# WestlyPark/StyleRenderer

Measured on AMD Instinct MI355X. Metric: generator fwd+bwd images/sec at 256^2, higher is better.
Workload: dtype f32

## Files before the change

stylerenderer_amd/csrc/conv1x1_gemm.h:

```cpp
#pragma once
#include <hip/hip_runtime.h>
#include <stdint.h>

bool sr_conv1x1_gemm_eligible(int64_t B, int64_t C, int64_t N, int64_t ldw, int64_t P, const void* in, const void* wt,
                              const void* out);
int sr_conv1x1_gemm_launch(float* out, const float* in, const float* wt, int64_t ldw, const float* iscale,
                           const float* oscale, const float* obias, int64_t B, int64_t C, int64_t N, int64_t P,
                           hipStream_t st, const float* addend = nullptr);

bool sr_convt_taps_gemm_eligible(int64_t B, int64_t C, int64_t N, int64_t IW, int64_t ldw, int c_per_slice,
                                 const void* wt);
int sr_convt_taps_gemm_launch(float* partial, const float* in, const float* wt, int64_t ldw, const float* iscale, int64_t B,
                              int64_t C, int64_t N, int64_t IH, int64_t IW, int ks, int c_per_slice, hipStream_t st);
```

stylerenderer_amd/csrc/conv1x1_gemm.hip:

```cpp
#include "mfma_tile.h"
#include "conv1x1_gemm.h"

#include <cstdlib>

namespace {

constexpr int TN = 128, TP = 128, KC = 16;

struct GemmParams {
    const float* x;
    const float* wt;
    const float* iscale;
    const float* oscale;
    const float* obias;
    const float* addend;
    float* out;
    int C, N, ldw;
    int64_t P;
    int tiles_p, tiles_n;
};

__global__ __launch_bounds__(256, 2) void k_conv1x1_gemm(const GemmParams q) {
#if __HIP_DEVICE_COMPILE__
    __shared__ float s_a[2][KC][TN];
    __shared__ float s_b[2][KC][TP];
    int bid = blockIdx.x;
    const int tp = bid % q.tiles_p;
    bid /= q.tiles_p;
    const int tn = bid % q.tiles_n;
    const int b = bid / q.tiles_n;
    const int n0 = tn * TN;
    const int64_t p0 = (int64_t)tp * TP;
    const int tid = threadIdx.x, lane = tid & 63, wave = tid >> 6;
    const int l31 = lane & 31, half = lane >> 5;
    const int wn = (wave >> 1) * 64, wp = (wave & 1) * 64;

    const int r0 = tid >> 5, c4 = (tid & 31) * 4;
    const float* wsrc = q.wt + (int64_t)r0 * q.ldw + n0 + c4;
    const float* xsrc = q.x + ((int64_t)b * q.C + r0) * q.P + p0 + c4;
    const float* isc = q.iscale ? q.iscale + (int64_t)b * q.C : nullptr;
    const int64_t wstep8 = (int64_t)8 * q.ldw, xstep8 = (int64_t)8 * q.P;

    f32x16 acc[2][2];
#pragma unroll
    for (int i = 0; i < 2; ++i)
#pragma unroll
        for (int j = 0; j < 2; ++j)
#pragma unroll
            for (int r = 0; r < 16; ++r) acc[i][j][r] = 0.0f;

    float4 ra0, ra1, rb0, rb1;
    auto fetch = [&](int kc) {
        const float* w = wsrc + (int64_t)kc * KC * q.ldw;
        const float* xx = xsrc + (int64_t)kc * KC * q.P;
        ra0 = *reinterpret_cast<const float4*>(w);
        ra1 = *reinterpret_cast<const float4*>(w + wstep8);
        rb0 = *reinterpret_cast<const float4*>(xx);
        rb1 = *reinterpret_cast<const float4*>(xx + xstep8);
        if (isc) {
            const float s0 = isc[kc * KC + r0], s1 = isc[kc * KC + r0 + 8];
            rb0.x *= s0; rb0.y *= s0; rb0.z *= s0; rb0.w *= s0;
            rb1.x *= s1; rb1.y *= s1; rb1.z *= s1; rb1.w *= s1;
        }
    };
    auto stash = [&](int buf) {
        *reinterpret_cast<float4*>(&s_a[buf][r0][c4]) = ra0;
        *reinterpret_cast<float4*>(&s_a[buf][r0 + 8][c4]) = ra1;
        *reinterpret_cast<float4*>(&s_b[buf][r0][c4]) = rb0;
        *reinterpret_cast<float4*>(&s_b[buf][r0 + 8][c4]) = rb1;
    };

    const int nchunks = q.C / KC;
    fetch(0);
    stash(0);
    __syncthreads();
    for (int kc = 0; kc < nchunks; ++kc) {
        const int buf = kc & 1;
        const bool more = kc + 1 < nchunks;
        if (more) fetch(kc + 1);
#pragma unroll
        for (int kk = 0; kk < KC / 2; ++kk) {
            const int k = 2 * kk + half;
            const float a0 = s_a[buf][k][wn + l31], a1 = s_a[buf][k][wn + 32 + l31];
            const float b0 = s_b[buf][k][wp + l31], b1 = s_b[buf][k][wp + 32 + l31];
            acc[0][0] = __builtin_amdgcn_mfma_f32_32x32x2f32(a0, b0, acc[0][0], 0, 0, 0);
            acc[0][1] = __builtin_amdgcn_mfma_f32_32x32x2f32(a0, b1, acc[0][1], 0, 0, 0);
            acc[1][0] = __builtin_amdgcn_mfma_f32_32x32x2f32(a1, b0, acc[1][0], 0, 0, 0);
            acc[1][1] = __builtin_amdgcn_mfma_f32_32x32x2f32(a1, b1, acc[1][1], 0, 0, 0);
        }
        if (more) stash(buf ^ 1);
        __syncthreads();
    }

    float* dst = q.out + ((int64_t)b * q.N + n0 + wn) * q.P + p0 + wp + l31;
    const float* osc = q.oscale ? q.oscale + (int64_t)b * q.N + n0 + wn : nullptr;
    const float* bia = q.obias ? q.obias + n0 + wn : nullptr;
#pragma unroll
    for (int i = 0; i < 2; ++i)
#pragma unroll
        for (int r = 0; r < 16; ++r) {
            const int row = sr_mfma32_row(r, half, i * 32);
            const float s = osc ? osc[row] : 1.0f;
            const float t = bia ? bia[row] : 0.0f;
            float* d = dst + (int64_t)row * q.P;
            float v0 = acc[i][0][r] * s + t, v1 = acc[i][1][r] * s + t;
            if (q.addend) {
                const float* a = q.addend + (d - q.out);
                v0 += a[0];
                v1 += a[32];
            }
            d[0] = v0;
            d[32] = v1;
        }
#endif
}

struct TapParams {
    const float* x;
    const float* wt;
    const float* iscale;
    float* partial;
    int B, C, N, ldw, IH, IW, GW, region;
    int tiles_q, tiles_n, c_per_slice;
    int64_t total_q;
};

__global__ __launch_bounds__(256, 2) void k_convt_taps_gemm(const TapParams q) {
#if __HIP_DEVICE_COMPILE__
    __shared__ float s_a[2][KC][TN];
    __shared__ float s_b[2][KC][TP];
    int bid = blockIdx.x;
    const int tap = bid % 9;
    bid /= 9;
    const int tn = bid % q.tiles_n;
    bid /= q.tiles_n;
    const int tq = bid % q.tiles_q;
    const int slice = bid / q.tiles_q;
    const int c_beg = slice * q.c_per_slice;
    const int c_end = min(q.C, c_beg + q.c_per_slice);
    const int n0 = tn * TN;
    const int tid = threadIdx.x, lane = tid & 63, wave = tid >> 6;
    const int l31 = lane & 31, half = lane >> 5;
    const int wn = (wave >> 1) * 64, wp = (wave & 1) * 64;
    const int ky = tap / 3, kx = tap - 3 * ky;

    const int r0 = tid >> 5, c4 = (tid & 31) * 4;
    const float* wsrc = q.wt + ((int64_t)tap * q.C + c_beg + r0) * q.ldw + n0 + c4;
    const int64_t wstep8 = (int64_t)8 * q.ldw;
    const int col = tid & 127, rb0 = tid >> 7;
    const int64_t qi = (int64_t)tq * TP + col;
    const int plane = q.IH * q.IW;
    bool ok = qi < q.total_q;
    const int bq = ok ? (int)(qi / q.region) : 0;
    const int g = ok ? (int)(qi - (int64_t)bq * q.region) : 0;
    const int yy = g / q.GW - (ky >> 1), xx = g % q.GW - (kx >> 1);
    ok = ok && yy >= 0 && yy < q.IH && xx >= 0 && xx < q.IW;
    const float* xsrc = q.x + ((int64_t)bq * q.C + c_beg + rb0) * plane + (ok ? yy * q.IW + xx : 0);
    const float* isc = q.iscale ? q.iscale + (int64_t)bq * q.C + c_beg + rb0 : nullptr;

    f32x16 acc[2][2];
#pragma unroll
    for (int i = 0; i < 2; ++i)
#pragma unroll
        for (int j = 0; j < 2; ++j)
#pragma unroll
            for (int r = 0; r < 16; ++r) acc[i][j][r] = 0.0f;

    float4 ra0, ra1;
    float rb[8];
    auto fetch = [&](int kc) {
        const float* w = wsrc + (int64_t)kc * KC * q.ldw;
        ra0 = *reinterpret_cast<const float4*>(w);
        ra1 = *reinterpret_cast<const float4*>(w + wstep8);
        const float* xx_ = xsrc + (int64_t)kc * KC * plane;
#pragma unroll
        for (int i = 0; i < 8; ++i) {
            float v = ok ? xx_[(int64_t)(2 * i) * plane] : 0.0f;
            if (isc) v *= isc[kc * KC + 2 * i];
            rb[i] = v;
        }
    };
    auto stash = [&](int buf) {
        *reinterpret_cast<float4*>(&s_a[buf][r0][c4]) = ra0;
        *reinterpret_cast<float4*>(&s_a[buf][r0 + 8][c4]) = ra1;
#pragma unroll
        for (int i = 0; i < 8; ++i) s_b[buf][rb0 + 2 * i][col] = rb[i];
    };

    const int nchunks = (c_end - c_beg) / KC;
    if (nchunks > 0) {
        fetch(0);
        stash(0);
    }
    __syncthreads();
    for (int kc = 0; kc < nchunks; ++kc) {
        const int buf = kc & 1;
        const bool more = kc + 1 < nchunks;
        if (more) fetch(kc + 1);
#pragma unroll
        for (int kk = 0; kk < KC / 2; ++kk) {
            const int k = 2 * kk + half;
            const float a0 = s_a[buf][k][wn + l31], a1 = s_a[buf][k][wn + 32 + l31];
            const float b0 = s_b[buf][k][wp + l31], b1 = s_b[buf][k][wp + 32 + l31];
            acc[0][0] = __builtin_amdgcn_mfma_f32_32x32x2f32(a0, b0, acc[0][0], 0, 0, 0);
            acc[0][1] = __builtin_amdgcn_mfma_f32_32x32x2f32(a0, b1, acc[0][1], 0, 0, 0);
            acc[1][0] = __builtin_amdgcn_mfma_f32_32x32x2f32(a1, b0, acc[1][0], 0, 0, 0);
            acc[1][1] = __builtin_amdgcn_mfma_f32_32x32x2f32(a1, b1, acc[1][1], 0, 0, 0);
        }
        if (more) stash(buf ^ 1);
        __syncthreads();
    }

    float* base = q.partial + ((int64_t)slice * 9 + tap) * q.B * q.N * q.region;
#pragma unroll
    for (int j = 0; j < 2; ++j) {
        const int64_t qo = (int64_t)tq * TP + wp + j * 32 + l31;
        if (qo >= q.total_q) continue;
        const int bo = (int)(qo / q.region);
        const int go = (int)(qo - (int64_t)bo * q.region);
        float* d = base + ((int64_t)bo * q.N + n0 + wn) * q.region + go;
#pragma unroll
        for (int i = 0; i < 2; ++i)
#pragma unroll
            for (int r = 0; r < 16; ++r) {
                const int row = sr_mfma32_row(r, half, i * 32);
                d[(int64_t)row * q.region] = acc[i][j][r];
            }
    }
#endif
}

int mode() {
    const int e = sr_env_char("SR_CONV1X1_GEMM");
    return e == '0' ? 0 : (e == 'f' ? 2 : 1);
}

}

bool sr_conv1x1_gemm_eligible(int64_t B, int64_t C, int64_t N, int64_t ldw, int64_t P, const void* in, const void* wt,
                              const void* out) {
    const int m = mode();
    if (m == 0 || B <= 0) return false;
    if (C % KC != 0 || N % TN != 0 || P % TP != 0 || ldw % 4 != 0) return false;
    if (((reinterpret_cast<uintptr_t>(in) | reinterpret_cast<uintptr_t>(wt) | reinterpret_cast<uintptr_t>(out)) & 15) != 0)
        return false;
    const int64_t tiles = (P / TP) * (N / TN) * B;
    return (m == 2 || tiles >= SR_NUM_CU) && tiles < (1LL << 31);
}

int sr_conv1x1_gemm_launch(float* out, const float* in, const float* wt, int64_t ldw, const float* iscale,
                           const float* oscale, const float* obias, int64_t B, int64_t C, int64_t N, int64_t P,
                           hipStream_t st, const float* addend) {
    GemmParams q;
    q.x = in; q.wt = wt; q.iscale = iscale; q.oscale = oscale; q.obias = obias; q.out = out; q.addend = addend;
    q.C = (int)C; q.N = (int)N; q.ldw = (int)ldw; q.P = P;
    q.tiles_p = (int)(P / TP); q.tiles_n = (int)(N / TN);
    const int64_t tiles = (int64_t)q.tiles_p * q.tiles_n * B;
    hipLaunchKernelGGL(k_conv1x1_gemm, dim3((unsigned)tiles), dim3(256), 0, st, q);
    return sr_launch_status();
}

bool sr_convt_taps_gemm_eligible(int64_t B, int64_t C, int64_t N, int64_t IW, int64_t ldw, int c_per_slice,
                                 const void* wt) {
    const int e = sr_env_char("SR_CONVT_TAPS_GEMM");
    if (e == '0') return false;
    if (IW > 32 && e != 'f') return false;
    return B > 0 && C % KC == 0 && c_per_slice % KC == 0 && N % TN == 0 && ldw % 4 == 0 &&
           (reinterpret_cast<uintptr_t>(wt) & 15) == 0;
}

int sr_convt_taps_gemm_launch(float* partial, const float* in, const float* wt, int64_t ldw, const float* iscale, int64_t B,
                              int64_t C, int64_t N, int64_t IH, int64_t IW, int ks, int c_per_slice, hipStream_t st) {
    TapParams q;
    q.x = in; q.wt = wt; q.iscale = iscale; q.partial = partial;
    q.B = (int)B; q.C = (int)C; q.N = (int)N; q.ldw = (int)ldw; q.IH = (int)IH; q.IW = (int)IW;
    q.GW = (int)IW + 1; q.region = (int)((IH + 1) * (IW + 1));
    q.total_q = B * q.region;
    q.tiles_q = (int)((q.total_q + TP - 1) / TP); q.tiles_n = (int)(N / TN); q.c_per_slice = c_per_slice;
    const int64_t blocks = (int64_t)q.tiles_q * q.tiles_n * 9 * ks;
    if (blocks > 0x7FFFFFFFLL) return SR_ERANGE;
    hipLaunchKernelGGL(k_convt_taps_gemm, dim3((unsigned)blocks), dim3(256), 0, st, q);
    return sr_launch_status();
}

extern "C" int sr_conv1x1_add_supported(int64_t B, int64_t C, int64_t N, int64_t wt_ld, int64_t P, const float* in,
                                        const float* wt, const float* out, const float* addend) {
    return sr_conv1x1_gemm_eligible(B, C, N, wt_ld, P, in, wt, out) && (reinterpret_cast<uintptr_t>(addend) & 15) == 0 ? 1 : 0;
}

extern "C" int sr_conv1x1_add(float* out, const float* in, const float* wt, const float* oscale, const float* addend,
                              int64_t B, int64_t C, int64_t N, int64_t wt_ld, int64_t P, sr_stream_t stream) {
    if (!out || !in || !wt || !addend) return SR_EINVAL;
    if (!sr_conv1x1_add_supported(B, C, N, wt_ld, P, in, wt, out, addend)) return SR_EINVAL;
    if (B * C * P >= (1LL << 31)) return SR_ERANGE;
    return sr_conv1x1_gemm_launch(out, in, wt, wt_ld, nullptr, oscale, nullptr, B, C, N, P, sr_stream(stream), addend);
}
```

stylerenderer_amd/csrc/conv_mfma.hip:

```cpp
#include "conv_mfma.h"

#include "conv1x1_gemm.h"
#include "mfma_tile.h"

#include <algorithm>
#include <cstdlib>

namespace {

constexpr int BN = 128;
constexpr int BM = 128;

__device__ __attribute__((aligned(16))) const float g_zero_line[4] = {0.f, 0.f, 0.f, 0.f};
__device__ __attribute__((aligned(16))) const float g_ones_line[4] = {1.f, 1.f, 1.f, 1.f};

template <int IS, int TY, int TX, int PW, int PH, int PB, bool V4, bool TAP9 = false>
struct Geo {
    static constexpr bool ROT = V4 && IS == 2;
    static constexpr int NT = TY * TX;
    static constexpr int KC = NT >= 9 ? 4 : (NT >= 4 ? 8 : 16);
    static constexpr int EH = (PH - 1) * IS + TY;
    static constexpr int EW = (PW - 1) * IS + TX;
    static constexpr int LEAD = (V4 && !ROT) ? (TAP9 ? 4 : (TX > 1 ? 3 : 0)) : 0;
    static constexpr int EWP = ROT ? (EW + 3 + 3) / 4 * 4
                                   : (V4 ? (LEAD + EW + 3) / 4 * 4 : EW + ((EW % 2 == 0) ? 1 : 0));
    static constexpr int PLANE = PB * EH * EWP;
    static constexpr int W_FLOATS = NT * KC * BN;
    static constexpr int W_INSTR = W_FLOATS / 256;
    static constexpr int IMG_INSTR = V4 ? (KC * PLANE + 255) / 256 : 0;
    static constexpr int ST_INSTR = V4 ? (KC * PB + 63) / 64 : 0;
    static constexpr int IN_FLOATS = KC * PLANE + KC * PB;
    static constexpr int IN_INSTR = V4 ? IMG_INSTR + ST_INSTR : (IN_FLOATS + 63) / 64;
    static constexpr int S_BASE = V4 ? W_FLOATS + IMG_INSTR * 256 : W_FLOATS + KC * PLANE;
    static constexpr int BUF = V4 ? S_BASE + ST_INSTR * 64 : W_FLOATS + IN_INSTR * 64;
    static constexpr int W_PER_WAVE = (W_INSTR + 3) / 4;
    static constexpr int IN_PER_WAVE = (IN_INSTR + 3) / 4;
    static constexpr int LDS_BYTES = 2 * BUF * 4;
};

template <int IS, int TY, int TX, int PW, int PH, int PB, bool V4, bool FAST, bool TAP9 = false>
__global__ __launch_bounds__(256) void k_conv_mfma(const ConvParams p) {
    using G = Geo<IS, TY, TX, PW, PH, PB, V4, TAP9>;
    static_assert(PW * PH * PB == BM, "patch must hold 128 pixels");
    static_assert(!TAP9 || (IS == 1 && TY == 1 && TX == 1), "tap-split mode is a shifted 1x1 convolution");
    extern __shared__ __attribute__((aligned(16))) float smem[];

    int bid = sr_xcd_chunk(blockIdx.x, gridDim.x);
    int tap = 0, g_dy0 = p.dy0, g_dx0 = p.dx0, g_gh = p.GH, g_gw = p.GW, g_ooy = p.ooy, g_oox = p.oox, g_slab = p.wmap[0];
    int tap_local = 0;
    if (TAP9) {
        tap_local = bid % p.tap_count;
        bid /= p.tap_count;
        tap = p.tap_first + tap_local * p.tap_step;
        const int ky = tap / 3, kx = tap - 3 * ky;
        g_dy0 = -(ky >> 1); g_dx0 = -(kx >> 1);
        g_ooy = ky & 1; g_oox = kx & 1;
        g_gh = min(g_ooy ? p.IH : p.IH + 1, p.GH); g_gw = min(g_oox ? p.IW : p.IW + 1, p.GW);
        g_slab = tap;
    }
    const SrTile tile = sr_tile_decode(bid, p.tiles_n, p.tiles_x, p.tiles_y);
    const int tb_i = tile.rest % p.tiles_b;
    const int slice = tile.rest / p.tiles_b;
    const int c_beg = slice * p.c_per_slice;
    const int c_end = min(p.C, c_beg + p.c_per_slice);
    const int n0 = tile.n_t * BN, gy0 = p.gy_base + tile.ty * PH, gx0 = p.gx_base + tile.tx * PW, b0 = tb_i * PB;
    const int iy0 = gy0 * IS + g_dy0, ix0 = gx0 * IS + g_dx0;

    const int tid = threadIdx.x, lane = tid & 63;
    const int wave = __builtin_amdgcn_readfirstlane(tid >> 6);
    const int half = lane >> 5, l31 = lane & 31;
    const int wco = wave & 1, wpx = wave >> 1;

    int a_off[2], b_off[2], s_off[2];
    int b_rot[2][4];
#pragma unroll
    for (int t = 0; t < 2; ++t) {
        a_off[t] = half * BN + wco * 64 + t * 32 + l31;
        const int m = wpx * 64 + t * 32 + l31;
        const int px = m % PW, py = (m / PW) % PH, pb = m / (PW * PH);
        b_off[t] = G::W_FLOATS + half * G::PLANE + (pb * G::EH + py * IS) * G::EWP + px * IS + G::LEAD +
                   ((TAP9 && V4) ? g_dx0 : 0);
        s_off[t] = G::S_BASE + pb * G::KC + half;
        const int l0 = half + iy0 + py * IS + ix0;
#pragma unroll
        for (int k = 0; k < 4; ++k) b_rot[t][k] = b_off[t] + ((l0 + k) & 3);
    }

    int w_src[G::W_PER_WAVE];
    int w_cl[G::W_PER_WAVE];
#pragma unroll
    for (int i = 0; i < G::W_PER_WAVE; ++i) {
        const int j = wave + 4 * i;
        const int row = 2 * j + half;
        const int t = row / G::KC, c = row % G::KC;
        const int col = min(n0 + l31 * 4, p.ldw - 4);
        w_cl[i] = (j < G::W_INSTR) ? c : -1;
        int slab = 0;
#pragma unroll
        for (int k = 0; k < G::NT; ++k)
            if (t == k) slab = p.wmap[k];
        if (TAP9) slab = g_slab;
        w_src[i] = (slab * p.C + c) * p.ldw + col;
    }
    int i_src[G::IN_PER_WAVE];
    int i_cl[G::IN_PER_WAVE];
#pragma unroll
    for (int i = 0; i < G::IN_PER_WAVE; ++i) {
        const int j = wave + 4 * i;
        int src = -1, c = 0, pb = 0;
        if (V4) {
            const int f = (j * 64 + lane) * 4;
            if (j < G::IMG_INSTR && f < G::KC * G::PLANE) {
                c = f / G::PLANE;
                const int q = f % G::PLANE;
                const int cola = q % G::EWP, r = (q / G::EWP) % G::EH;
                pb = q / (G::EWP * G::EH);
                const int gy = iy0 + r;
                int gx = ((TAP9 && V4) ? gx0 : ix0) - G::LEAD + cola;
                bool ok = gy >= 0 && gy < p.IH && b0 + pb < p.B;
                if (G::ROT) {
                    gx = ix0 - ((c * (p.IH * p.IW) + gy * p.IW + ix0) & 3) + cola;
                } else {
                    ok = ok && gx >= 0 && gx + 3 < p.IW;
                }
                if (ok) src = (pb * p.C + c) * p.IH * p.IW + gy * p.IW + gx;
            } else if (j >= G::IMG_INSTR && j < G::IN_INSTR) {
                const int e = (j - G::IMG_INSTR) * 64 + lane;
                if (e < G::KC * PB) {
                    pb = e / G::KC;
                    c = e % G::KC;
                    src = -2;
                }
            }
        } else {
            const int f = j * 64 + lane;
            if (j < G::IN_INSTR && f < G::KC * G::PLANE) {
                c = f / G::PLANE;
                const int q = f % G::PLANE;
                const int colp = q % G::EWP, r = (q / G::EWP) % G::EH;
                pb = q / (G::EWP * G::EH);
                const int gy = iy0 + r, gx = ix0 + colp;
                if (colp < G::EW && gy >= 0 && gy < p.IH && gx >= 0 && gx < p.IW && b0 + pb < p.B)
                    src = (pb * p.C + c) * p.IH * p.IW + gy * p.IW + gx;
            } else if (j < G::IN_INSTR && f < G::IN_FLOATS) {
                const int e = f - G::KC * G::PLANE;
                pb = e / G::KC;
                c = e % G::KC;
                src = -2;
            }
        }
        i_src[i] = src;
        i_cl[i] = c | (pb << 8);
    }
    const float* in_base = p.in + (int64_t)b0 * p.C * p.IH * p.IW;
    const int plane_in = p.IH * p.IW;

    const char* f_wp[G::W_PER_WAVE];
    const char* f_ip[G::IN_PER_WAVE];
    unsigned f_is[G::IN_PER_WAVE];
    if (FAST) {
#pragma unroll
        for (int i = 0; i < G::W_PER_WAVE; ++i) f_wp[i] = reinterpret_cast<const char*>(p.wt + w_src[i]);
#pragma unroll
        for (int i = 0; i < G::IN_PER_WAVE; ++i) {
            const int c = i_cl[i] & 255, pb = i_cl[i] >> 8;
            const char* ptr = reinterpret_cast<const char*>(g_zero_line);
            unsigned str = 0;
            if (i_src[i] >= 0) {
                ptr = reinterpret_cast<const char*>(in_base + i_src[i]);
                str = (unsigned)plane_in * 4u;
            } else if (i_src[i] == -2) {
                const bool ok = p.iscale && b0 + pb < p.B;
                ptr = ok ? reinterpret_cast<const char*>(p.iscale + (int64_t)(b0 + pb) * p.C + c)
                         : reinterpret_cast<const char*>(g_ones_line);
                str = ok ? 4u : 0u;
            }
            f_ip[i] = ptr;
            f_is[i] = str;
        }
    }
    const unsigned w_chunk_stride = (unsigned)p.ldw * 4u;

    auto dma = [&](int c0, int buf) {
        float* dst = smem + buf * G::BUF;
        if (FAST) {
#pragma unroll
            for (int i = 0; i < G::W_PER_WAVE; ++i) {
                const int j = wave + 4 * i;
                if (j < G::W_INSTR)
                    __builtin_amdgcn_global_load_lds((gptr_t)(f_wp[i] + (uint64_t)(unsigned)c0 * w_chunk_stride),
                                                     (lptr_t)(dst + j * 256), 16, 0, 0);
            }
#pragma unroll
            for (int i = 0; i < G::IN_PER_WAVE; ++i) {
                const int j = wave + 4 * i;
                if (j < G::IN_INSTR) {
                    const char* src = f_ip[i] + (uint64_t)(unsigned)c0 * f_is[i];
                    if (V4 && j < G::IMG_INSTR)
                        __builtin_amdgcn_global_load_lds((gptr_t)src, (lptr_t)(dst + G::W_FLOATS + j * 256), 16, 0, 0);
                    else if (V4)
                        __builtin_amdgcn_global_load_lds((gptr_t)src,
                                                         (lptr_t)(dst + G::S_BASE + (j - G::IMG_INSTR) * 64), 4, 0, 0);
                    else
                        __builtin_amdgcn_global_load_lds((gptr_t)src, (lptr_t)(dst + G::W_FLOATS + j * 64), 4, 0, 0);
                }
            }
            return;
        }
#pragma unroll
        for (int i = 0; i < G::W_PER_WAVE; ++i) {
            const int j = wave + 4 * i;
            if (j < G::W_INSTR) {
                const float* src = (c0 + w_cl[i] < p.C) ? p.wt + w_src[i] + (int64_t)c0 * p.ldw : g_zero_line;
                __builtin_amdgcn_global_load_lds((gptr_t)src, (lptr_t)(dst + j * 256), 16, 0, 0);
            }
        }
#pragma unroll
        for (int i = 0; i < G::IN_PER_WAVE; ++i) {
            const int j = wave + 4 * i;
            if (j < G::IN_INSTR) {
                const int c = i_cl[i] & 255, pb = i_cl[i] >> 8;
                const bool c_ok = c0 + c < p.C;
                const float* src = g_zero_line;
                if (i_src[i] >= 0 && c_ok) src = in_base + i_src[i] + (int64_t)c0 * plane_in;
                if (i_src[i] == -2)
                    src = (p.iscale && c_ok && b0 + pb < p.B) ? p.iscale + (int64_t)(b0 + pb) * p.C + c0 + c
                                                              : g_ones_line;
                if (V4 && j < G::IMG_INSTR)
                    __builtin_amdgcn_global_load_lds((gptr_t)src, (lptr_t)(dst + G::W_FLOATS + j * 256), 16, 0, 0);
                else if (V4)
                    __builtin_amdgcn_global_load_lds((gptr_t)src,
                                                     (lptr_t)(dst + G::S_BASE + (j - G::IMG_INSTR) * 64), 4, 0, 0);
                else
                    __builtin_amdgcn_global_load_lds((gptr_t)src, (lptr_t)(dst + G::W_FLOATS + j * 64), 4, 0, 0);
            }
        }
    };

    f32x16 acc[2][2];
#pragma unroll
    for (int i = 0; i < 2; ++i)
#pragma unroll
        for (int j = 0; j < 2; ++j)
#pragma unroll
            for (int r = 0; r < 16; ++r) acc[i][j][r] = 0.0f;

    dma(c_beg, 0);
    int buf = 0;
    for (int c0 = c_beg; c0 < c_end; c0 += G::KC) {
        __syncthreads();
        if (c0 + G::KC < c_end) dma(c0 + G::KC, buf ^ 1);
        const float* sb = smem + buf * G::BUF;
#pragma unroll
        for (int cp = 0; cp < G::KC / 2; ++cp) {
            const float sc0 = sb[s_off[0] + 2 * cp];
            const float sc1 = (PB > 1) ? sb[s_off[1] + 2 * cp] : sc0;
#pragma unroll
            for (int ty = 0; ty < TY; ++ty)
#pragma unroll
                for (int tx = 0; tx < TX; ++tx) {
                    const int w_tap = ((ty * TX + tx) * G::KC + 2 * cp) * BN;
                    const int i_tap = (2 * cp) * G::PLANE + ty * G::EWP + tx;
                    float a0 = sb[w_tap + a_off[0]];
                    float a1 = sb[w_tap + a_off[1]];
                    float x0 = sb[i_tap + (G::ROT ? b_rot[0][(2 * cp + ty) & 3] : b_off[0])];
                    float x1 = sb[i_tap + (G::ROT ? b_rot[1][(2 * cp + ty) & 3] : b_off[1])];
                    if (PB == 1) { a0 *= sc0; a1 *= sc0; }
                    else { x0 *= sc0; x1 *= sc1; }
                    acc[0][0] = __builtin_amdgcn_mfma_f32_32x32x2f32(a0, x0, acc[0][0], 0, 0, 0);
                    acc[0][1] = __builtin_amdgcn_mfma_f32_32x32x2f32(a0, x1, acc[0][1], 0, 0, 0);
                    acc[1][0] = __builtin_amdgcn_mfma_f32_32x32x2f32(a1, x0, acc[1][0], 0, 0, 0);
                    acc[1][1] = __builtin_amdgcn_mfma_f32_32x32x2f32(a1, x1, acc[1][1], 0, 0, 0);
                }
        }
        buf ^= 1;
    }

    const int64_t plane_out = (int64_t)p.OH * p.OW;
#pragma unroll
    for (int pt = 0; pt < 2; ++pt) {
        const int m = wpx * 64 + pt * 32 + l31;
        const int px = m % PW, py = (m / PW) % PH, pb = m / (PW * PH);
        const int gy = gy0 + py, gx = gx0 + px, b = b0 + pb;
        if (gy >= g_gh || gx >= g_gw || b >= p.B) continue;
        const int64_t pix = (int64_t)(gy * p.osy + g_ooy) * p.OW + (gx * p.osx + g_oox);
#pragma unroll
        for (int ct = 0; ct < 2; ++ct)
#pragma unroll
            for (int r = 0; r < 16; ++r) {
                const int n = sr_mfma32_row(r, half, n0 + wco * 64 + ct * 32);
                if (n < p.N) {
                    float v = acc[ct][pt][r];
                    if (TAP9) {
                        const int rw = p.GW - p.gx_base, rh = p.GH - p.gy_base;
                        p.partial[((((int64_t)slice * p.tap_count + tap_local) * p.B + b) * p.N + n) * (rh * rw) +
                                  (gy - p.gy_base) * rw + (gx - p.gx_base)] = v;
                    } else if (p.ks > 1) {
                        const int rw = p.GW - p.gx_base, rh = p.GH - p.gy_base;
                        p.partial[(((int64_t)slice * p.B + b) * p.N + n) * (rh * rw) +
                                  (gy - p.gy_base) * rw + (gx - p.gx_base)] = v;
                    } else {
                        if (p.oscale) v *= p.oscale[(int64_t)b * p.N + n];
                        if (p.obias) v += p.obias[n];
                        p.out[((int64_t)b * p.N + n) * plane_out + pix] = v;
                    }
                }
            }
    }
}

template <int IS, int TY, int TX, int PW, int PH, int PB, bool V4, bool FAST, bool TAP9 = false>
int launch_fast(const ConvParams& p, dim3 grid, hipStream_t st) {
    using G = Geo<IS, TY, TX, PW, PH, PB, V4, TAP9>;
    constexpr auto kern = k_conv_mfma<IS, TY, TX, PW, PH, PB, V4, FAST, TAP9>;
    if (!sr_allow_dynamic_lds<kern>(G::LDS_BYTES)) return SR_EINVAL;
    hipLaunchKernelGGL(kern, grid, dim3(256), G::LDS_BYTES, st, p);
    return sr_launch_status();
}

template <int IS, int TY, int TX, int PW, int PH, int PB, bool V4, bool TAP9 = false>
int launch_one(const ConvParams& p, dim3 grid, hipStream_t st) {
    using G = Geo<IS, TY, TX, PW, PH, PB, V4, TAP9>;
    if (p.C % G::KC == 0 && p.c_per_slice % G::KC == 0)
        return launch_fast<IS, TY, TX, PW, PH, PB, V4, true, TAP9>(p, grid, st);
    return launch_fast<IS, TY, TX, PW, PH, PB, V4, false, TAP9>(p, grid, st);
}

void patch_shape(int GW, int& pw, int& ph, int& pb) {
    if (GW > 16) { pw = 32; ph = 4; pb = 1; }
    else if (GW > 8) { pw = 16; ph = 8; pb = 1; }
    else if (GW > 4) { pw = 8; ph = 8; pb = 2; }
    else { pw = 4; ph = 4; pb = 8; }
}

void choose_split(int GH, int GW, int B, int N, int C, int& ks, int& c_per_slice) {
    int pw, ph, pb;
    patch_shape(GW, pw, ph, pb);
    const int64_t blocks = (int64_t)((GW + pw - 1) / pw) * ((GH + ph - 1) / ph) * ((B + pb - 1) / pb) *
                           ((N + BN - 1) / BN);
    ks = 1;
    c_per_slice = (C + 15) / 16 * 16;
    if (blocks >= SR_NUM_CU || C < 64) return;
    int want = (int)((2 * SR_NUM_CU + blocks - 1) / blocks);
    if (want > 16) want = 16;
    int per = (C + want - 1) / want;
    per = (per + 15) / 16 * 16;
    if (per < 32) per = 32;
    c_per_slice = per;
    ks = (C + per - 1) / per;
}

__global__ __launch_bounds__(256) void k_conv_reduce(const ConvParams p, int rh, int rw) {
    const int64_t region = (int64_t)rh * rw, total = (int64_t)p.B * p.N * region;
    const int64_t plane_out = (int64_t)p.OH * p.OW;
    for (int64_t i = (int64_t)blockIdx.x * blockDim.x + threadIdx.x; i < total;
         i += (int64_t)gridDim.x * blockDim.x) {
        float acc = 0.0f;
#pragma unroll 8
        for (int s = 0; s < p.ks; ++s) acc += p.partial[s * total + i];
        const int64_t row = i / region;
        const int q = (int)(i - row * region);
        const int gy = p.gy_base + q / rw, gx = p.gx_base + q % rw;
        if (p.oscale) acc *= p.oscale[row];
        if (p.obias) acc += p.obias[row % p.N];
        p.out[row * plane_out + (int64_t)(gy * p.osy + p.ooy) * p.OW + (gx * p.osx + p.oox)] = acc;
    }
}

__global__ __launch_bounds__(256) void k_convt_tap_reduce(const ConvParams p) {
    const int rh = p.GH, rw = p.GW;
    const int64_t region = (int64_t)rh * rw, plane_out = (int64_t)p.OH * p.OW;
    const int64_t total = (int64_t)p.B * p.N * plane_out, slab = (int64_t)p.B * p.N * region;
    for (int64_t i = (int64_t)blockIdx.x * blockDim.x + threadIdx.x; i < total;
         i += (int64_t)gridDim.x * blockDim.x) {
        const int64_t row = i / plane_out;
        const int q = (int)(i - row * plane_out);
        const int Y = q / p.OW, X = q - Y * p.OW;
        const int py = Y & 1, px = X & 1;
        const int64_t at = row * region + (int64_t)(Y >> 1) * rw + (X >> 1);
        float acc = 0.0f;
        for (int s = 0; s < p.ks; ++s)
            for (int ky = py; ky < 3; ky += 2)
                for (int kx = px; kx < 3; kx += 2) acc += p.partial[((int64_t)s * 9 + ky * 3 + kx) * slab + at];
        if (p.oscale) acc *= p.oscale[row];
        if (p.obias) acc += p.obias[row % p.N];
        p.out[i] = acc;
    }
}

bool taps_v4(const ConvParams& p) {
    return !sr_env_off("SR_CONVT_TAPS_V4") && p.IW % 4 == 0 && p.gx_base % 4 == 0 && sr_aligned16(p.in);
}

__global__ __launch_bounds__(256) void k_convt_strip_reduce(const ConvParams p, const float* __restrict__ prow,
                                                            const float* __restrict__ pcol, int ks_row, int ks_col) {
    const int rw = p.IW + 1, ch = p.IH, OW = p.OW, OH = p.OH;
    const int per_row = OW + OH - 1;
    const int64_t planes = (int64_t)p.B * p.N, total = planes * per_row;
    for (int64_t i = (int64_t)blockIdx.x * blockDim.x + threadIdx.x; i < total;
         i += (int64_t)gridDim.x * blockDim.x) {
        const int64_t row = i / per_row;
        const int q = (int)(i - row * per_row);
        float acc;
        int64_t o;
        acc = 0.0f;
        if (q < OW) {
            const int g = q >> 1;
            const float* t = prow + row * rw + g;
            for (int s = 0; s < ks_row; ++s, t += 3 * planes * rw)
                acc += (q & 1) ? t[planes * rw] : t[0] + t[2 * planes * rw];
            o = (int64_t)(OH - 1) * OW + q;
        } else {
            const int Y = q - OW, g = Y >> 1;
            const float* t = pcol + row * ch + g;
            for (int s = 0; s < ks_col; ++s, t += 3 * planes * ch)
                acc += (Y & 1) ? t[planes * ch] : t[0] + t[2 * planes * ch];
            o = (int64_t)Y * OW + (OW - 1);
        }
        if (p.oscale) acc *= p.oscale[row];
        if (p.obias) acc += p.obias[row % p.N];
        p.out[row * (int64_t)OH * OW + o] = acc;
    }
}

constexpr int STRIP_KS = 4;

template <int PW, int PH, int PB>
int launch_strip_part(ConvParams& p, hipStream_t st) {
    p.tiles_x = (p.GW - p.gx_base + PW - 1) / PW;
    p.tiles_y = (p.GH - p.gy_base + PH - 1) / PH;
    p.tiles_b = (p.B + PB - 1) / PB;
    p.tiles_n = (p.N + BN - 1) / BN;
    int64_t blocks = (int64_t)p.tiles_x * p.tiles_y * p.tiles_b * p.tiles_n * p.tap_count;
    p.ks = 1; p.c_per_slice = (p.C + 15) / 16 * 16;
    for (int ks = STRIP_KS; ks >= 2; ks /= 2)
        if (p.C % (16 * ks) == 0 && p.C / ks >= 64 && blocks * ks <= 4 * SR_NUM_CU) {
            p.ks = ks;
            p.c_per_slice = p.C / ks;
            break;
        }
    blocks *= p.ks;
    if (blocks > 0x7FFFFFFFLL) return SR_ERANGE;
    if (PB == 1 && taps_v4(p)) return launch_one<1, 1, 1, PW, PH, PB, PB == 1, true>(p, dim3((unsigned)blocks), st);
    return launch_one<1, 1, 1, PW, PH, PB, false, true>(p, dim3((unsigned)blocks), st);
}

template <int IS, int TY, int TX>
int launch_by_patch(ConvParams& p, hipStream_t st) {
    int pw, ph, pb;
    const int ext_w = p.GW - p.gx_base, ext_h = p.GH - p.gy_base;
    if (ext_w <= 0 || ext_h <= 0) return SR_OK;
    choose_split(ext_h, ext_w, p.B, p.N, p.C, p.ks, p.c_per_slice);
    if (!p.partial || (int64_t)p.ks * p.B * p.N * ext_h * ext_w > p.partial_floats) {
        p.ks = 1;
        p.c_per_slice = (p.C + 15) / 16 * 16;
    }
    patch_shape(ext_w, pw, ph, pb);
    p.tiles_x = (ext_w + pw - 1) / pw;
    p.tiles_y = (ext_h + ph - 1) / ph;
    p.tiles_b = (p.B + pb - 1) / pb;
    p.tiles_n = (p.N + BN - 1) / BN;
    const int64_t blocks = (int64_t)p.tiles_x * p.tiles_y * p.tiles_b * p.tiles_n * p.ks;
    if (blocks <= 0) return SR_OK;
    if (blocks > 0x7FFFFFFFLL) return SR_ERANGE;
    const dim3 grid((unsigned)blocks);
    const bool v4 = IS == 1 && pb == 1 && p.IW % 4 == 0 && sr_aligned16(p.in) &&
                    p.gx_base % 4 == 0 && p.dx0 == (TX > 1 ? -1 : 0);
    const bool rot = IS == 2 && pb == 1 && (p.IW & 3) == 1 && ((p.IH * p.IW) & 3) == 1 && p.C % 4 == 0 &&
                     sr_aligned16(p.in) && p.dx0 >= 0 && p.dy0 >= 0 && p.gx_base == 0 &&
                     p.gy_base == 0 && (p.GW - 1) * 2 + p.dx0 + TX <= p.IW && (p.GH - 1) * 2 + p.dy0 + TY <= p.IH &&
                     ext_w % pw == 0 && ext_h % ph == 0 && !sr_env_off("SR_CONV_ROT");
    int rc;
    if (IS == 1 && v4) {
        if (pw == 32) rc = launch_one<1, TY, TX, 32, 4, 1, true>(p, grid, st);
        else rc = launch_one<1, TY, TX, 16, 8, 1, true>(p, grid, st);
    } else if (IS == 2 && rot && TY == 3 && TX == 3) {
        if (pw == 32) rc = launch_one<2, 3, 3, 32, 4, 1, true>(p, grid, st);
        else rc = launch_one<2, 3, 3, 16, 8, 1, true>(p, grid, st);
    } else if (pw == 32) rc = launch_one<IS, TY, TX, 32, 4, 1, false>(p, grid, st);
    else if (pw == 16) rc = launch_one<IS, TY, TX, 16, 8, 1, false>(p, grid, st);
    else if (pw == 8) rc = launch_one<IS, TY, TX, 8, 8, 2, false>(p, grid, st);
    else rc = launch_one<IS, TY, TX, 4, 4, 8, false>(p, grid, st);
    if (rc != SR_OK || p.ks <= 1) return rc;
    const int64_t total = (int64_t)p.B * p.N * ext_h * ext_w;
    hipLaunchKernelGGL(k_conv_reduce, dim3(sr_stream_grid(total, 256)), dim3(256), 0, st, p, ext_h, ext_w);
    return sr_launch_status();
}

}


int64_t sr_conv_direct_floats(int64_t B, int64_t C, int64_t N, int64_t IH, int64_t IW, int64_t OH, int64_t OW,
                              int transposed) {
    int ks, per;
    int64_t need = 0;
    auto consider = [&](int64_t gh, int64_t gw) {
        if (gh <= 0 || gw <= 0) return;
        choose_split((int)gh, (int)gw, (int)B, (int)N, (int)C, ks, per);
        if (ks > 1) need = std::max(need, ks * B * N * gh * gw);
    };
    if (!transposed) consider(OH, OW);
    else consider(IH + 1, IW + 1), consider(IH, IW), consider(1, IW + 1), consider(IH, 1);
    return need;
}

int sr_conv_direct_launch(ConvParams p, int ksize, int stride, int pad, hipStream_t st) {
    p.GH = p.OH; p.GW = p.OW;
    p.gy_base = p.gx_base = 0;
    p.osy = p.osx = 1; p.ooy = p.oox = 0;
    p.dy0 = p.dx0 = -pad;
    for (int i = 0; i < ksize * ksize; ++i) p.wmap[i] = i;
    if (ksize == 3) return stride == 1 ? launch_by_patch<1, 3, 3>(p, st) : launch_by_patch<2, 3, 3>(p, st);
    return stride == 1 ? launch_by_patch<1, 1, 1>(p, st) : launch_by_patch<2, 1, 1>(p, st);
}

void sr_convt_taps_plan(int IH, int IW, int B, int N, int C, int& ks, int& c_per_slice) {
    if (sr_convt_taps_gemm_eligible(B, C, N, IW, 4, 16, nullptr)) {
        const int64_t tiles = sr_ceil_div((int64_t)B * (IH + 1) * (IW + 1), 128) * (N / 128) * 9;
        static const int per_cu = [] {
            const char* e = std::getenv("SR_TAPS_WGS");
            const int v = e ? std::atoi(e) : 0;
            return v >= 1 && v <= 8 ? v : 2;
        }();
        int want = (int)sr_ceil_div((int64_t)per_cu * SR_NUM_CU, tiles);
        if (want > 8) want = 8;
        if (want < 1) want = 1;
        int per = (C + want - 1) / want;
        per = (per + 15) / 16 * 16;
        if (per < 64) per = 64;
        if (per > C) per = C;
        c_per_slice = per;
        ks = (C + per - 1) / per;
        return;
    }
    int pw, ph, pb;
    patch_shape(IW + 1, pw, ph, pb);
    const int64_t blocks = (int64_t)((IW + pw) / pw) * ((IH + ph) / ph) * ((B + pb - 1) / pb) * ((N + BN - 1) / BN) * 9;
    ks = 1;
    c_per_slice = (C + 15) / 16 * 16;
    if (blocks >= 2 * SR_NUM_CU || C < 64) return;
    int want = (int)((2 * SR_NUM_CU + blocks - 1) / blocks);
    if (want > 8) want = 8;
    int per = (C + want - 1) / want;
    per = (per + 15) / 16 * 16;
    if (per < 32) per = 32;
    c_per_slice = per;
    ks = (C + per - 1) / per;
}

bool sr_convt_taps_wanted(int64_t B, int64_t C, int64_t N, int64_t IH, int64_t IW) {
    const int sw = sr_env_char("SR_CONVT_TAPS");
    if (sw >= 0) return sw != '0';
    return 18.0 * (double)B * (double)C * (double)N * (double)IH * (double)IW < 1.05e10;
}

int sr_convt_taps_launch(ConvParams p, int ks, int c_per_slice, bool gemm, hipStream_t st) {
    p.GH = p.IH + 1; p.GW = p.IW + 1;
    p.gy_base = p.gx_base = 0;
    p.osy = p.osx = 2; p.ooy = p.oox = 0;
    p.dy0 = p.dx0 = 0;
    p.tap_first = 0; p.tap_step = 1; p.tap_count = 9;
    p.ks = ks; p.c_per_slice = c_per_slice;
    int pw, ph, pb;
    patch_shape(p.GW, pw, ph, pb);
    p.tiles_x = (p.GW + pw - 1) / pw;
    p.tiles_y = (p.GH + ph - 1) / ph;
    p.tiles_b = (p.B + pb - 1) / pb;
    p.tiles_n = (p.N + BN - 1) / BN;
    const int64_t blocks = (int64_t)p.tiles_x * p.tiles_y * p.tiles_b * p.tiles_n * p.ks * 9;
    if (blocks > 0x7FFFFFFFLL) return SR_ERANGE;
    const dim3 grid((unsigned)blocks);
    const bool v4 = taps_v4(p);
    int rc;
    if (gemm)
        rc = sr_convt_taps_gemm_launch(p.partial, p.in, p.wt, p.ldw, p.iscale, p.B, p.C, p.N, p.IH, p.IW, p.ks, p.c_per_slice, st);
    else if (pw == 32) rc = v4 ? launch_one<1, 1, 1, 32, 4, 1, true, true>(p, grid, st)
                          : launch_one<1, 1, 1, 32, 4, 1, false, true>(p, grid, st);
    else if (pw == 16) rc = v4 ? launch_one<1, 1, 1, 16, 8, 1, true, true>(p, grid, st)
                               : launch_one<1, 1, 1, 16, 8, 1, false, true>(p, grid, st);
    else if (pw == 8) rc = launch_one<1, 1, 1, 8, 8, 2, false, true>(p, grid, st);
    else rc = launch_one<1, 1, 1, 4, 4, 8, false, true>(p, grid, st);
    if (rc != SR_OK) return rc;
    const int64_t total = (int64_t)p.B * p.N * p.OH * p.OW;
    hipLaunchKernelGGL(k_convt_tap_reduce, dim3(sr_stream_grid(total, 256)), dim3(256), 0, st, p);
    return sr_launch_status();
}

int64_t sr_convt_strip_floats(int64_t B, int64_t N, int64_t IH, int64_t IW) { return STRIP_KS * 3 * B * N * (IW + 1 + IH); }

int sr_convt_strips_launch(ConvParams p, hipStream_t st) {
    float* prow = p.partial;
    float* pcol = p.partial + STRIP_KS * 3 * (int64_t)p.B * p.N * (p.IW + 1);
    p.osy = p.osx = 2; p.ooy = p.oox = 0;
    p.dy0 = p.dx0 = 0;
    p.ks = 1; p.c_per_slice = (p.C + 15) / 16 * 16;
    p.gy_base = p.IH; p.GH = p.IH + 1; p.gx_base = 0; p.GW = p.IW + 1;
    p.tap_first = 6; p.tap_step = 1; p.tap_count = 3;
    p.partial = prow;
    int rc = launch_strip_part<32, 4, 1>(p, st);
    if (rc != SR_OK) return rc;
    const int ks_row = p.ks;
    p.gy_base = 0; p.GH = p.IH; p.gx_base = p.IW; p.GW = p.IW + 1;
    p.tap_first = 2; p.tap_step = 3; p.tap_count = 3;
    p.partial = pcol;
    rc = launch_strip_part<4, 4, 8>(p, st);
    if (rc != SR_OK) return rc;
    const int ks_col = p.ks;
    const int64_t total = (int64_t)p.B * p.N * (p.OW + p.OH - 1);
    hipLaunchKernelGGL(k_convt_strip_reduce, dim3(sr_stream_grid(total, 256)), dim3(256), 0, st, p, prow, pcol, ks_row,
                       ks_col);
    return sr_launch_status();
}

int sr_convt_phases_launch(ConvParams p, bool interior_done, hipStream_t st) {
    for (int py = 0; py < 2; ++py)
        for (int px = 0; px < 2; ++px) {
            const int TYp = py == 0 ? 2 : 1, TXp = px == 0 ? 2 : 1;
            p.osy = p.osx = 2; p.ooy = py; p.oox = px;
            p.dy0 = -(TYp - 1); p.dx0 = -(TXp - 1);
            for (int ty = 0; ty < TYp; ++ty)
                for (int tx = 0; tx < TXp; ++tx) {
                    const int ky = py + 2 * (TYp - 1 - ty), kx = px + 2 * (TXp - 1 - tx);
                    p.wmap[ty * TXp + tx] = ky * 3 + kx;
                }
            const int gh_full = py == 0 ? p.IH + 1 : p.IH, gw_full = px == 0 ? p.IW + 1 : p.IW;
            int regions[3][4] = {{0, p.IH, 0, p.IW},
                                 {p.IH, gh_full, 0, gw_full},
                                 {0, p.IH, p.IW, gw_full}};
            const bool split_border = p.IW >= 16;
            if (!split_border) {
                regions[0][1] = gh_full;
                regions[0][3] = gw_full;
            }
            const bool fused = split_border && interior_done;
            for (int rg = fused ? 1 : 0; rg < (split_border ? 3 : 1); ++rg) {
                p.gy_base = regions[rg][0]; p.GH = regions[rg][1];
                p.gx_base = regions[rg][2]; p.GW = regions[rg][3];
                if (p.GH <= p.gy_base || p.GW <= p.gx_base) continue;
                int rc;
                if (py == 0 && px == 0) rc = launch_by_patch<1, 2, 2>(p, st);
                else if (py == 0) rc = launch_by_patch<1, 2, 1>(p, st);
                else if (px == 0) rc = launch_by_patch<1, 1, 2>(p, st);
                else rc = launch_by_patch<1, 1, 1>(p, st);
                if (rc != SR_OK) return rc;
            }
        }
    return SR_OK;
}
```

Baseline: 634.8.

## Fuse transposed-conv edge strips into one MFMA GEMM kernel launch

Adds a dedicated MFMA GEMM kernel that computes both the bottom-row and right-column edge strips of the stride-2 transposed convolution in a single launch. It replaces the two separate generic tap-conv launches, with input scaling folded into the operand loads. The strip reduce kernel is rewritten to use a non-grid-stride layout with 32-bit indexing, with explicit range checks added. This targets launch overhead and poor utilisation on small edge regions, at the cost of more code paths and masked loads for ragged tiles.

```diff
diff --git a/stylerenderer_amd/csrc/conv1x1_gemm.h b/stylerenderer_amd/csrc/conv1x1_gemm.h
--- a/stylerenderer_amd/csrc/conv1x1_gemm.h
+++ b/stylerenderer_amd/csrc/conv1x1_gemm.h
@@ -12,3 +12,8 @@
                                  const void* wt);
 int sr_convt_taps_gemm_launch(float* partial, const float* in, const float* wt, int64_t ldw, const float* iscale, int64_t B,
                               int64_t C, int64_t N, int64_t IH, int64_t IW, int ks, int c_per_slice, hipStream_t st);
+
+bool sr_convt_strip_gemm_eligible(int64_t B, int64_t N, int64_t IH, int64_t IW, int64_t ldw, const void* wt);
+int sr_convt_strip_gemm_launch(float* prow, float* pcol, const float* in, const float* wt, int64_t ldw, const float* iscale,
+                               int64_t B, int64_t C, int64_t N, int64_t IH, int64_t IW, int ks_row, int cps_row, int ks_col,
+                               int cps_col, hipStream_t st);
diff --git a/stylerenderer_amd/csrc/conv1x1_gemm.hip b/stylerenderer_amd/csrc/conv1x1_gemm.hip
--- a/stylerenderer_amd/csrc/conv1x1_gemm.hip
+++ b/stylerenderer_amd/csrc/conv1x1_gemm.hip
@@ -1,6 +1,7 @@
 #include "mfma_tile.h"
 #include "conv1x1_gemm.h"
 
+#include <algorithm>
 #include <cstdlib>
 
 namespace {
@@ -230,6 +231,151 @@
 #endif
 }
 
+struct StripParams {
+    const float* x;
+    const float* wt;
+    const float* iscale;
+    float* prow;
+    float* pcol;
+    int B, C, N, ldw, IH, IW, tiles_n;
+    int row_blocks, row_tiles, row_cps, row_span;
+    int col_tiles, col_cps;
+};
+
+__global__ __launch_bounds__(256, 2) void k_convt_strip_gemm(const StripParams q) {
+#if __HIP_DEVICE_COMPILE__
+    __shared__ float s_a[2][KC][TN];
+    __shared__ float s_b[2][KC][TP];
+    __shared__ float s_s[2][KC][4];
+    int bid = blockIdx.x;
+    const bool row = bid < q.row_blocks;
+    if (!row) bid -= q.row_blocks;
+    const int tiles_q = row ? q.row_tiles : q.col_tiles;
+    const int cps = row ? q.row_cps : q.col_cps;
+    const int span = row ? q.row_span : q.IH;
+    const int npts = row ? q.IW + 1 : q.IH;
+    const int t = bid % 3;
+    bid /= 3;
+    const int tn = bid % q.tiles_n;
+    bid /= q.tiles_n;
+    const int tq = bid % tiles_q;
+    const int slice = bid / tiles_q;
+    const int tap = row ? 6 + t : 2 + 3 * t;
+    const int c_beg = slice * cps;
+    const int c_len = min(q.C, c_beg + cps) - c_beg;
+    const int n0 = tn * TN;
+    const int tid = threadIdx.x, lane = tid & 63, wave = tid >> 6;
+    const int l31 = lane & 31, half = lane >> 5;
+    const int wn = (wave >> 1) * 64, wp = (wave & 1) * 64;
+
+    const int r0 = tid >> 5, c4 = (tid & 31) * 4;
+    const float* wsrc = q.wt + ((int64_t)tap * q.C + c_beg + r0) * q.ldw + min(n0 + c4, q.ldw - 4);
+    const int64_t wstep8 = (int64_t)8 * q.ldw;
+    const int col = tid & 127, rb0 = tid >> 7;
+    const int qi = tq * TP + col;
+    const int plane = q.IH * q.IW;
+    const int bq = qi / span, g = qi - bq * span;
+    const int along = g - (t >> 1);
+    const bool ok = bq < q.B && g < npts && along >= 0 && along < (row ? q.IW : q.IH);
+    const int at = row ? (q.IH - 1) * q.IW + along : along * q.IW + q.IW - 1;
+    const float* xsrc = q.x + ((int64_t)(ok ? bq : 0) * q.C + c_beg + rb0) * plane + (ok ? at : 0);
+    const float* isc = (!row && q.iscale && ok) ? q.iscale + (int64_t)bq * q.C + c_beg + rb0 : nullptr;
+    const int sk = (tid >> 2) & 15, sg = tid & 3;
+    const int sb = (tq * TP + sg * 32) / span;
+    const float* ssrc = (row && q.iscale && tid < 64 && sb < q.B) ? q.iscale + (int64_t)sb * q.C + c_beg + sk : nullptr;
+
+    f32x16 acc[2][2];
+#pragma unroll
+    for (int i = 0; i < 2; ++i)
+#pragma unroll
+        for (int j = 0; j < 2; ++j)
+#pragma unroll
+            for (int r = 0; r < 16; ++r) acc[i][j][r] = 0.0f;
+
+    struct Stage {
+        float4 ra0, ra1;
+        float rb[8], rx[8], rs;
+    };
+    auto fetch = [&](int kc, Stage& g) {
+        const int k0 = kc * KC;
+        const float* w = wsrc + (int64_t)k0 * q.ldw;
+        g.ra0 = *reinterpret_cast<const float4*>(k0 + r0 < c_len ? w : q.wt);
+        g.ra1 = *reinterpret_cast<const float4*>(k0 + r0 + 8 < c_len ? w + wstep8 : q.wt);
+        const float* xx_ = xsrc + (int64_t)k0 * plane;
+#pragma unroll
+        for (int i = 0; i < 8; ++i) {
+            const bool in = ok && k0 + rb0 + 2 * i < c_len;
+            g.rb[i] = *(in ? xx_ + (int64_t)(2 * i) * plane : q.x);
+            g.rx[i] = *((isc && in) ? isc + k0 + 2 * i : q.x);
+        }
+        g.rs = *((ssrc && k0 + sk < c_len) ? ssrc + k0 : q.x);
+    };
+    auto stash = [&](int kc, const Stage& g) {
+        const int buf = kc & 1, k0 = kc * KC;
+        const bool in0 = k0 + r0 < c_len, in1 = k0 + r0 + 8 < c_len;
+        *reinterpret_cast<float4*>(&s_a[buf][r0][c4]) = in0 ? g.ra0 : make_float4(0.0f, 0.0f, 0.0f, 0.0f);
+        *reinterpret_cast<float4*>(&s_a[buf][r0 + 8][c4]) = in1 ? g.ra1 : make_float4(0.0f, 0.0f, 0.0f, 0.0f);
+#pragma unroll
+        for (int i = 0; i < 8; ++i) {
+            const bool in = ok && k0 + rb0 + 2 * i < c_len;
+            s_b[buf][rb0 + 2 * i][col] = !in ? 0.0f : (isc ? g.rb[i] * g.rx[i] : g.rb[i]);
+        }
+        if (tid < 64) s_s[buf][sk][sg] = (ssrc && k0 + sk < c_len) ? g.rs : 1.0f;
+    };
+    const int gsel = wp >> 5;
+    auto products = [&](int buf) {
+#pragma unroll
+        for (int kk = 0; kk < KC / 2; ++kk) {
+            const int k = 2 * kk + half;
+            const float a0 = s_a[buf][k][wn + l31], a1 = s_a[buf][k][wn + 32 + l31];
+            const float b0 = s_b[buf][k][wp + l31], b1 = s_b[buf][k][wp + 32 + l31];
+            const float s0 = s_s[buf][k][gsel], s1 = s_s[buf][k][gsel + 1];
+            acc[0][0] = __builtin_amdgcn_mfma_f32_32x32x2f32(a0 * s0, b0, acc[0][0], 0, 0, 0);
+            acc[0][1] = __builtin_amdgcn_mfma_f32_32x32x2f32(a0 * s1, b1, acc[0][1], 0, 0, 0);
+            acc[1][0] = __builtin_amdgcn_mfma_f32_32x32x2f32(a1 * s0, b0, acc[1][0], 0, 0, 0);
+            acc[1][1] = __builtin_amdgcn_mfma_f32_32x32x2f32(a1 * s1, b1, acc[1][1], 0, 0, 0);
+        }
+    };
+
+    const int nchunks = (c_len + KC - 1) / KC;
+    Stage g0, g1;
+    if (nchunks > 0) {
+        fetch(0, g0);
+        stash(0, g0);
+    }
+    if (nchunks > 0) fetch(min(1, nchunks - 1), g0);
+    __syncthreads();
+    const int last = nchunks - 1;
+    for (int kc = 0; kc < nchunks; kc += 2) {
+        fetch(min(kc + 2, last), g1);
+        products(0);
+        if (kc + 1 < nchunks) stash(kc + 1, g0);
+        __syncthreads();
+        if (kc + 1 >= nchunks) break;
+        fetch(min(kc + 3, last), g0);
+        products(1);
+        if (kc + 2 < nchunks) stash(kc + 2, g1);
+        __syncthreads();
+    }
+
+    float* base = (row ? q.prow : q.pcol) + ((int64_t)slice * 3 + t) * q.B * q.N * npts;
+#pragma unroll
+    for (int j = 0; j < 2; ++j) {
+        const int qo = tq * TP + wp + j * 32 + l31;
+        const int bo = qo / span, go = qo - bo * span;
+        if (bo >= q.B || go >= npts) continue;
+        float* d = base + ((int64_t)bo * q.N + n0 + wn) * npts + go;
+#pragma unroll
+        for (int i = 0; i < 2; ++i)
+#pragma unroll
+            for (int r = 0; r < 16; ++r) {
+                const int nr = sr_mfma32_row(r, half, i * 32);
+                if (n0 + wn + nr < q.N) d[(int64_t)nr * npts] = acc[i][j][r];
+            }
+    }
+#endif
+}
+
 int mode() {
     const int e = sr_env_char("SR_CONV1X1_GEMM");
     return e == '0' ? 0 : (e == 'f' ? 2 : 1);
@@ -283,6 +429,32 @@
     return sr_launch_status();
 }
 
+bool sr_convt_strip_gemm_eligible(int64_t B, int64_t N, int64_t IH, int64_t IW, int64_t ldw, const void* wt) {
+    if (sr_env_off("SR_CONVT_STRIPS_GEMM")) return false;
+    const int64_t row_span = (IW + 1 + 31) / 32 * 32;
+    return B > 0 && N > 0 && ldw % 4 == 0 && ldw >= 4 && (reinterpret_cast<uintptr_t>(wt) & 15) == 0 &&
+           B * std::max(row_span, IH) + TP < (1LL << 31);
+}
+
+int sr_convt_strip_gemm_launch(float* prow, float* pcol, const float* in, const float* wt, int64_t ldw, const float* iscale,
+                               int64_t B, int64_t C, int64_t N, int64_t IH, int64_t IW, int ks_row, int cps_row, int ks_col,
+                               int cps_col, hipStream_t st) {
+    StripParams q;
+    q.x = in; q.wt = wt; q.iscale = iscale; q.prow = prow; q.pcol = pcol;
+    q.B = (int)B; q.C = (int)C; q.N = (int)N; q.ldw = (int)ldw; q.IH = (int)IH; q.IW = (int)IW;
+    q.tiles_n = (int)((N + TN - 1) / TN);
+    q.row_span = (int)((IW + 1 + 31) / 32 * 32);
+    q.row_tiles = (int)((B * q.row_span + TP - 1) / TP);
+    q.col_tiles = (int)((B * IH + TP - 1) / TP);
+    q.row_cps = cps_row; q.col_cps = cps_col;
+    const int64_t row_blocks = (int64_t)q.row_tiles * q.tiles_n * 3 * ks_row;
+    const int64_t blocks = row_blocks + (int64_t)q.col_tiles * q.tiles_n * 3 * ks_col;
+    if (blocks > 0x7FFFFFFFLL) return SR_ERANGE;
+    q.row_blocks = (int)row_blocks;
+    hipLaunchKernelGGL(k_convt_strip_gemm, dim3((unsigned)blocks), dim3(256), 0, st, q);
+    return sr_launch_status();
+}
+
 extern "C" int sr_conv1x1_add_supported(int64_t B, int64_t C, int64_t N, int64_t wt_ld, int64_t P, const float* in,
                                         const float* wt, const float* out, const float* addend) {
     return sr_conv1x1_gemm_eligible(B, C, N, wt_ld, P, in, wt, out) && (reinterpret_cast<uintptr_t>(addend) & 15) == 0 ? 1 : 0;
diff --git a/stylerenderer_amd/csrc/conv_mfma.hip b/stylerenderer_amd/csrc/conv_mfma.hip
--- a/stylerenderer_amd/csrc/conv_mfma.hip
+++ b/stylerenderer_amd/csrc/conv_mfma.hip
@@ -394,44 +394,45 @@
 
 __global__ __launch_bounds__(256) void k_convt_strip_reduce(const ConvParams p, const float* __restrict__ prow,
                                                             const float* __restrict__ pcol, int ks_row, int ks_col) {
-    const int rw = p.IW + 1, ch = p.IH, OW = p.OW, OH = p.OH;
-    const int per_row = OW + OH - 1;
-    const int64_t planes = (int64_t)p.B * p.N, total = planes * per_row;
-    for (int64_t i = (int64_t)blockIdx.x * blockDim.x + threadIdx.x; i < total;
-         i += (int64_t)gridDim.x * blockDim.x) {
-        const int64_t row = i / per_row;
-        const int q = (int)(i - row * per_row);
-        float acc;
-        int64_t o;
-        acc = 0.0f;
-        if (q < OW) {
-            const int g = q >> 1;
-            const float* t = prow + row * rw + g;
-            for (int s = 0; s < ks_row; ++s, t += 3 * planes * rw)
-                acc += (q & 1) ? t[planes * rw] : t[0] + t[2 * planes * rw];
-            o = (int64_t)(OH - 1) * OW + q;
-        } else {
-            const int Y = q - OW, g = Y >> 1;
-            const float* t = pcol + row * ch + g;
-            for (int s = 0; s < ks_col; ++s, t += 3 * planes * ch)
-                acc += (Y & 1) ? t[planes * ch] : t[0] + t[2 * planes * ch];
-            o = (int64_t)Y * OW + (OW - 1);
-        }
-        if (p.oscale) acc *= p.oscale[row];
-        if (p.obias) acc += p.obias[row % p.N];
-        p.out[row * (int64_t)OH * OW + o] = acc;
-    }
+    const unsigned rw = p.IW + 1, ch = p.IH, OW = p.OW, OH = p.OH;
+    const unsigned planes = (unsigned)p.B * p.N;
+    const unsigned row_blocks = (planes * OW + 255u) / 256u;
+    unsigned row;
+    float acc = 0.0f;
+    int64_t o;
+    if (blockIdx.x < row_blocks) {
+        const unsigned i = blockIdx.x * 256u + threadIdx.x;
+        if (i >= planes * OW) return;
+        row = i / OW;
+        const unsigned q = i - row * OW;
+        const float* t = prow + (row * rw + (q >> 1));
+        for (int s = 0; s < ks_row; ++s, t += 3u * planes * rw)
+            acc += (q & 1) ? t[planes * rw] : t[0] + t[2u * planes * rw];
+        o = (int64_t)(OH - 1) * OW + q;
+    } else {
+        const unsigned i = (blockIdx.x - row_blocks) * 256u + threadIdx.x;
+        if (i >= planes * (OH - 1)) return;
+        row = i / (OH - 1);
+        const unsigned Y = i - row * (OH - 1);
+        const float* t = pcol + (row * ch + (Y >> 1));
+        for (int s = 0; s < ks_col; ++s, t += 3u * planes * ch)
+            acc += (Y & 1) ? t[planes * ch] : t[0] + t[2u * planes * ch];
+        o = (int64_t)Y * OW + (OW - 1);
+    }
+    if (p.oscale) acc *= p.oscale[row];
+    if (p.obias) acc += p.obias[row % (unsigned)p.N];
+    p.out[row * ((int64_t)OH * OW) + o] = acc;
 }
 
 constexpr int STRIP_KS = 4;
 
 template <int PW, int PH, int PB>
-int launch_strip_part(ConvParams& p, hipStream_t st) {
+int64_t strip_plan(ConvParams& p) {
     p.tiles_x = (p.GW - p.gx_base + PW - 1) / PW;
     p.tiles_y = (p.GH - p.gy_base + PH - 1) / PH;
     p.tiles_b = (p.B + PB - 1) / PB;
     p.tiles_n = (p.N + BN - 1) / BN;
-    int64_t blocks = (int64_t)p.tiles_x * p.tiles_y * p.tiles_b * p.tiles_n * p.tap_count;
+    const int64_t blocks = (int64_t)p.tiles_x * p.tiles_y * p.tiles_b * p.tiles_n * p.tap_count;
     p.ks = 1; p.c_per_slice = (p.C + 15) / 16 * 16;
     for (int ks = STRIP_KS; ks >= 2; ks /= 2)
         if (p.C % (16 * ks) == 0 && p.C / ks >= 64 && blocks * ks <= 4 * SR_NUM_CU) {
@@ -439,7 +440,11 @@
             p.c_per_slice = p.C / ks;
             break;
         }
-    blocks *= p.ks;
+    return blocks * p.ks;
+}
+
+template <int PW, int PH, int PB>
+int launch_strip_part(const ConvParams& p, int64_t blocks, hipStream_t st) {
     if (blocks > 0x7FFFFFFFLL) return SR_ERANGE;
     if (PB == 1 && taps_v4(p)) return launch_one<1, 1, 1, PW, PH, PB, PB == 1, true>(p, dim3((unsigned)blocks), st);
     return launch_one<1, 1, 1, PW, PH, PB, false, true>(p, dim3((unsigned)blocks), st);
@@ -593,22 +598,29 @@
     float* pcol = p.partial + STRIP_KS * 3 * (int64_t)p.B * p.N * (p.IW + 1);
     p.osy = p.osx = 2; p.ooy = p.oox = 0;
     p.dy0 = p.dx0 = 0;
-    p.ks = 1; p.c_per_slice = (p.C + 15) / 16 * 16;
-    p.gy_base = p.IH; p.GH = p.IH + 1; p.gx_base = 0; p.GW = p.IW + 1;
-    p.tap_first = 6; p.tap_step = 1; p.tap_count = 3;
-    p.partial = prow;
-    int rc = launch_strip_part<32, 4, 1>(p, st);
+    const int64_t planes = (int64_t)p.B * p.N;
+    if (sr_convt_strip_floats(p.B, p.N, p.IH, p.IW) >= (1LL << 31) || planes * (p.OW + p.OH) >= (1LL << 31)) return SR_ERANGE;
+    ConvParams r = p;
+    r.gy_base = p.IH; r.GH = p.IH + 1; r.gx_base = 0; r.GW = p.IW + 1;
+    r.tap_first = 6; r.tap_step = 1; r.tap_count = 3;
+    r.partial = prow;
+    const int64_t row_blocks = strip_plan<32, 4, 1>(r);
+    ConvParams c = p;
+    c.gy_base = 0; c.GH = p.IH; c.gx_base = p.IW; c.GW = p.IW + 1;
+    c.tap_first = 2; c.tap_step = 3; c.tap_count = 3;
+    c.partial = pcol;
+    const int64_t col_blocks = strip_plan<4, 4, 8>(c);
+    int rc;
+    if (sr_convt_strip_gemm_eligible(p.B, p.N, p.IH, p.IW, p.ldw, p.wt)) {
+        rc = sr_convt_strip_gemm_launch(prow, pcol, p.in, p.wt, p.ldw, p.iscale, p.B, p.C, p.N, p.IH, p.IW, r.ks,
+                                        r.c_per_slice, c.ks, c.c_per_slice, st);
+    } else {
+        rc = launch_strip_part<32, 4, 1>(r, row_blocks, st);
+        if (rc == SR_OK) rc = launch_strip_part<4, 4, 8>(c, col_blocks, st);
+    }
     if (rc != SR_OK) return rc;
-    const int ks_row = p.ks;
-    p.gy_base = 0; p.GH = p.IH; p.gx_base = p.IW; p.GW = p.IW + 1;
-    p.tap_first = 2; p.tap_step = 3; p.tap_count = 3;
-    p.partial = pcol;
-    rc = launch_strip_part<4, 4, 8>(p, st);
-    if (rc != SR_OK) return rc;
-    const int ks_col = p.ks;
-    const int64_t total = (int64_t)p.B * p.N * (p.OW + p.OH - 1);
-    hipLaunchKernelGGL(k_convt_strip_reduce, dim3(sr_stream_grid(total, 256)), dim3(256), 0, st, p, prow, pcol, ks_row,
-                       ks_col);
+    const int64_t blocks = sr_ceil_div(planes * p.OW, 256) + sr_ceil_div(planes * (p.OH - 1), 256);
+    hipLaunchKernelGGL(k_convt_strip_reduce, dim3((unsigned)blocks), dim3(256), 0, st, p, prow, pcol, r.ks, c.ks);
     return sr_launch_status();
 }
 
```

New measurement: 637.3 (median of 6 runs). No clear change (+0.4%).
